# riffusion/riffusion-hobby

Measured on NVIDIA H100. Metric: clips/sec, higher is better.
Workload: dtype f16

## Files before the change

riffusion-hobby_b200/csrc/rf_attn.cu:

```cuda
#include <cuda.h>
#include <cuda_fp16.h>
#include <cuda_runtime.h>

#include <string>

#include "rf_common.h"
#include "rf_tc.cuh"

namespace {

constexpr int TQ = 128;
constexpr int TK = 64;
constexpr int ATTN_THREADS = 256 + 32;

struct AttnParams {
    int Nq, Nk, d, heads;
    int n_tiles;
    float c;
    __half* out;
    long out_pitch;
    int causal;
};

__device__ __forceinline__ uint32_t pack_half2(float a, float b) {
    const __half2 h = __floats2half2_rn(a, b);
    return *reinterpret_cast<const uint32_t*>(&h);
}
__device__ __forceinline__ float ex2(float a) {
    float r;
    asm("ex2.approx.ftz.f32 %0, %1;" : "=f"(r) : "f"(a));
    return r;
}

template <int DPAD, int NV, int NS>
__global__ void __launch_bounds__(ATTN_THREADS, 1)
k_flash_attn(const __grid_constant__ CUtensorMap mapQ, const __grid_constant__ CUtensorMap mapK,
             const __grid_constant__ CUtensorMap mapVt, const AttnParams p) {
    extern __shared__ __align__(1024) uint8_t smem[];
    rf_pdl_trigger();
    constexpr int NSLAB = DPAD / 64;
    constexpr int Q_BYTES = NSLAB * TQ * 128;
    constexpr int K_BYTES = NSLAB * TK * 128;
    constexpr int V_BYTES = ((NV * 128 + 1023) / 1024) * 1024;
    uint8_t* sQ = smem;
    uint8_t* sK = sQ + Q_BYTES;
    uint8_t* sV = sK + NS * K_BYTES;
    uint64_t* bars = reinterpret_cast<uint64_t*>(sV + NS * V_BYTES);
    uint64_t* q_full = bars;
    uint64_t* kv_full = bars + 1;
    uint64_t* kv_empty = kv_full + NS;

    const int warp = threadIdx.x >> 5, lane = threadIdx.x & 31;
    const int q_blk = blockIdx.x, head = blockIdx.y, b = blockIdx.z;
    const int T = p.n_tiles;

    if (threadIdx.x == 0) {
        tc::mbar_init(q_full, 1);
        for (int i = 0; i < NS; ++i) {
            tc::mbar_init(&kv_full[i], 1);
            tc::mbar_init(&kv_empty[i], 256);
        }
        tc::fence_barrier_init();
    }
    __syncthreads();
    rf_pdl_wait();

    if (warp == 8) {
        if (lane != 0) return;
        tc::mbar_expect_tx(q_full, Q_BYTES);
#pragma unroll
        for (int s = 0; s < NSLAB; ++s) tc::tma_load_4d(&mapQ, q_full, sQ + s * TQ * 128, s * 64, q_blk * TQ, head, b);
        for (int j = 0; j < T; ++j) {
            const int st = j % NS;
            tc::mbar_wait(&kv_empty[st], ((j / NS) & 1) ^ 1);
            tc::mbar_expect_tx(&kv_full[st], K_BYTES + NV * 128);
#pragma unroll
            for (int s = 0; s < NSLAB; ++s)
                tc::tma_load_4d(&mapK, &kv_full[st], sK + st * K_BYTES + s * TK * 128, s * 64, j * TK, head, b);
            tc::tma_load_4d(&mapVt, &kv_full[st], sV + st * V_BYTES, j * TK, 0, head, b);
        }
        return;
    }

    const int wg = warp >> 2;
    const int frag_row = wg * 64 + (warp & 3) * 16 + (lane >> 2), frag_col = 2 * (lane & 3);
    const int q0 = q_blk * TQ + frag_row, q1 = q0 + 8;
    const float c = p.c;
    float o[NV / 2];
#pragma unroll
    for (int i = 0; i < NV / 2; ++i) o[i] = 0.f;
    float m0 = -INFINITY, m1 = -INFINITY, l0 = 0.f, l1 = 0.f;
    const uint32_t q_base = tc::smem_u32(sQ) + wg * (64 * 128);
    tc::mbar_wait(q_full, 0);
    for (int j = 0; j < T; ++j) {
        const int st = j % NS;
        tc::mbar_wait(&kv_full[st], (j / NS) & 1);
        float s[TK / 2];
        const uint32_t k_base = tc::smem_u32(sK + st * K_BYTES);
        tc::wgmma_fence();
#pragma unroll
        for (int kk = 0; kk < DPAD / 16; ++kk) {
            const int sl = kk >> 2, k = kk & 3;
            tc::wgmma_ss<TK>(s, tc::make_desc_sw128(q_base + sl * TQ * 128 + k * 32),
                             tc::make_desc_sw128(k_base + sl * TK * 128 + k * 32), kk > 0 ? 1u : 0u);
        }
        tc::wgmma_commit();
        tc::wgmma_wait<0>();
        tc::reg_fence<TK / 2>(s);
        const int kmax0 = p.causal ? min(p.Nk, q0 + 1) : p.Nk, kmax1 = p.causal ? min(p.Nk, q1 + 1) : p.Nk;
        float mt0 = -INFINITY, mt1 = -INFINITY;
#pragma unroll
        for (int i = 0; i < TK / 8; ++i) {
#pragma unroll
            for (int e = 0; e < 2; ++e) {
                const int key = j * TK + 8 * i + frag_col + e;
                if (key >= kmax0) s[4 * i + e] = -INFINITY;
                if (key >= kmax1) s[4 * i + 2 + e] = -INFINITY;
                mt0 = fmaxf(mt0, s[4 * i + e]);
                mt1 = fmaxf(mt1, s[4 * i + 2 + e]);
            }
        }
        mt0 = fmaxf(mt0, __shfl_xor_sync(0xffffffffu, mt0, 1));
        mt0 = fmaxf(mt0, __shfl_xor_sync(0xffffffffu, mt0, 2));
        mt1 = fmaxf(mt1, __shfl_xor_sync(0xffffffffu, mt1, 1));
        mt1 = fmaxf(mt1, __shfl_xor_sync(0xffffffffu, mt1, 2));
        const float mn0 = fmaxf(m0, mt0), mn1 = fmaxf(m1, mt1);
        const float r0 = mn0 == -INFINITY ? 0.f : mn0, r1 = mn1 == -INFINITY ? 0.f : mn1;
        const float f0 = ex2((m0 - r0) * c), f1 = ex2((m1 - r1) * c);
        m0 = mn0;
        m1 = mn1;
        l0 *= f0;
        l1 *= f1;
#pragma unroll
        for (int i = 0; i < NV / 8; ++i) {
            o[4 * i] *= f0;
            o[4 * i + 1] *= f0;
            o[4 * i + 2] *= f1;
            o[4 * i + 3] *= f1;
        }
        const float mc0 = r0 * c, mc1 = r1 * c;
        uint32_t pa[TK / 4];
#pragma unroll
        for (int i = 0; i < TK / 8; ++i) {
            const uint32_t h0 = pack_half2(ex2(fmaf(s[4 * i], c, -mc0)), ex2(fmaf(s[4 * i + 1], c, -mc0)));
            const uint32_t h1 = pack_half2(ex2(fmaf(s[4 * i + 2], c, -mc1)), ex2(fmaf(s[4 * i + 3], c, -mc1)));
            const float2 g0 = __half22float2(*reinterpret_cast<const __half2*>(&h0));
            const float2 g1 = __half22float2(*reinterpret_cast<const __half2*>(&h1));
            l0 += g0.x + g0.y;
            l1 += g1.x + g1.y;
            pa[2 * i] = h0;
            pa[2 * i + 1] = h1;
        }
        const uint32_t v_base = tc::smem_u32(sV + st * V_BYTES);
        tc::wgmma_fence();
#pragma unroll
        for (int kk = 0; kk < TK / 16; ++kk)
            tc::wgmma_rs<NV>(o, pa + 4 * kk, tc::make_desc_sw128(v_base + kk * 32), 1u);
        tc::wgmma_commit();
        tc::wgmma_wait<0>();
        tc::reg_fence<NV / 2>(o);
        tc::mbar_arrive(&kv_empty[st]);
    }
    l0 += __shfl_xor_sync(0xffffffffu, l0, 1);
    l0 += __shfl_xor_sync(0xffffffffu, l0, 2);
    l1 += __shfl_xor_sync(0xffffffffu, l1, 1);
    l1 += __shfl_xor_sync(0xffffffffu, l1, 2);
    const float inv0 = 1.f / l0, inv1 = 1.f / l1;
    __half* dst0 = p.out + (static_cast<long>(b) * p.Nq + q0) * p.out_pitch + head * p.d;
    __half* dst1 = dst0 + 8 * p.out_pitch;
#pragma unroll
    for (int i = 0; i < NV / 8; ++i) {
        const int col = 8 * i + frag_col;
        if (col < p.d) {
            if (q0 < p.Nq) *reinterpret_cast<uint32_t*>(dst0 + col) = pack_half2(o[4 * i] * inv0, o[4 * i + 1] * inv0);
            if (q1 < p.Nq) *reinterpret_cast<uint32_t*>(dst1 + col) = pack_half2(o[4 * i + 2] * inv1, o[4 * i + 3] * inv1);
        }
    }
}

template <int DPAD, int NV, int NS>
int launch_attn(const CUtensorMap& mq, const CUtensorMap& mk, const CUtensorMap& mv, const AttnParams& p, dim3 grid,
                cudaStream_t st) {
    constexpr int NSLAB = DPAD / 64;
    constexpr int V_BYTES = ((NV * 128 + 1023) / 1024) * 1024;
    constexpr size_t smem = static_cast<size_t>(NSLAB) * TQ * 128 + static_cast<size_t>(NS) * (NSLAB * TK * 128 + V_BYTES) +
                            256 + 1024;
    static_assert(smem <= 232448, "shared memory budget (227 KB per block)");
    static rf_dev_once once;
    const cudaError_t aerr = rf_set_smem_once(once, k_flash_attn<DPAD, NV, NS>, int(smem));
    if (aerr != cudaSuccess) return rf_fail(RF_ERR_CUDA, std::string("cudaFuncSetAttribute(k_flash_attn): ") + cudaGetErrorString(aerr));
    RF_LAUNCH_PDL("k_flash_attn", (k_flash_attn<DPAD, NV, NS>), grid, dim3(ATTN_THREADS), smem, st,
                  grid.x * grid.y * grid.z <= 600u, mq, mk, mv, p);
    return RF_OK;
}

}

extern "C" int rf_attention_masked_f16(const void* q, const void* k, const void* vt, void* out, int B, int heads, int Nq,
                                       int Nk, int d, int vt_pitch, float scale, int causal, void* stream) {
    if (causal && (Nk > 128 || d > 112))
        return rf_fail(RF_ERR_UNSUPPORTED, "rf_attention_masked_f16: the causal mask is implemented for Nk <= 128, d <= 112 "
                                           "(the 77-token text encoder)");
    if (!q || !k || !vt || !out || B <= 0 || heads <= 0 || Nq <= 0 || Nk <= 0 || d <= 0 || (d % 8) || vt_pitch < Nk ||
        (vt_pitch % 8))
        return rf_fail(RF_ERR_INVALID, "rf_attention_masked_f16: bad argument");
    if (d > 192) return rf_fail(RF_ERR_UNSUPPORTED, "rf_attention_masked_f16: head dim > 192 (use the GEMM + softmax path)");
    const long C = static_cast<long>(heads) * d;
    const int es[4] = {1, 1, 1, 1};
    CUtensorMap mq, mk, mv;
    {
        const long dims[4] = {d, Nq, heads, B};
        const long str[4] = {1, C, d, static_cast<long>(Nq) * C};
        const int box[4] = {64, TQ, 1, 1};
        int rc = rf_tma_map_f16(&mq, q, dims, str, box, es);
        if (rc) return rc;
    }
    {
        const long dims[4] = {d, Nk, heads, B};
        const long str[4] = {1, C, d, static_cast<long>(Nk) * C};
        const int box[4] = {64, TK, 1, 1};
        int rc = rf_tma_map_f16(&mk, k, dims, str, box, es);
        if (rc) return rc;
    }
    const int NV = d <= 48 ? 48 : d <= 64 ? 64 : d <= 80 ? 80 : d <= 96 ? 96 : d <= 112 ? 112 : d <= 128 ? 128 : d <= 160 ? 160 : 192;
    {
        const long dims[4] = {Nk, d, heads, B};
        const long str[4] = {1, vt_pitch, static_cast<long>(d) * vt_pitch, C * vt_pitch};
        const int box[4] = {TK, NV, 1, 1};
        int rc = rf_tma_map_f16(&mv, vt, dims, str, box, es);
        if (rc) return rc;
    }
    AttnParams p;
    p.Nq = Nq; p.Nk = Nk; p.d = d; p.heads = heads;
    p.n_tiles = (Nk + TK - 1) / TK;
    p.c = scale * 1.4426950408889634f;
    p.out = static_cast<__half*>(out);
    p.out_pitch = C;
    p.causal = causal ? 1 : 0;
    dim3 grid((Nq + TQ - 1) / TQ, heads, B);
    cudaStream_t st = static_cast<cudaStream_t>(stream);
    if (d <= 48) return launch_attn<64, 48, 4>(mq, mk, mv, p, grid, st);
    if (d <= 64) return launch_attn<64, 64, 4>(mq, mk, mv, p, grid, st);
    if (d <= 80) return launch_attn<128, 80, 3>(mq, mk, mv, p, grid, st);
    if (d <= 96) return launch_attn<128, 96, 3>(mq, mk, mv, p, grid, st);
    if (d <= 112) return launch_attn<128, 112, 3>(mq, mk, mv, p, grid, st);
    if (d <= 128) return launch_attn<128, 128, 3>(mq, mk, mv, p, grid, st);
    if (d <= 160) return launch_attn<192, 160, 2>(mq, mk, mv, p, grid, st);
    return launch_attn<192, 192, 2>(mq, mk, mv, p, grid, st);
}
```

Measured before the change: 3.839.

## Parameterize flash attention by warpgroup count and skip padded head-dim work

The kernel is templated on head-dim max and the number of consumer warpgroups. Small head dims (<=64) now use 4 warpgroups and a 256-row Q tile, which halves K/V reloads per query. The QK^T k-loop now runs only up to the real head dim instead of the padded slab width, and masking runs only for causal or ragged tail tiles. The empty barrier now counts per-warp arrivals rather than per-thread ones. In exchange there are more registers and threads per block for small d, and fewer blocks in the grid.

```diff
diff --git a/riffusion-hobby_b200/csrc/rf_attn.cu b/riffusion-hobby_b200/csrc/rf_attn.cu
--- a/riffusion-hobby_b200/csrc/rf_attn.cu
+++ b/riffusion-hobby_b200/csrc/rf_attn.cu
@@ -9,9 +9,7 @@
 
 namespace {
 
-constexpr int TQ = 128;
 constexpr int TK = 64;
-constexpr int ATTN_THREADS = 256 + 32;
 
 struct AttnParams {
     int Nq, Nk, d, heads;
@@ -32,16 +30,30 @@
     return r;
 }
 
-template <int DPAD, int NV, int NS>
-__global__ void __launch_bounds__(ATTN_THREADS, 1)
+template <int DMAX, int NWG, int NS>
+struct AttnCfg {
+    static constexpr int TQ = 64 * NWG;
+    static constexpr int THREADS = 128 * NWG + 32;
+    static constexpr int NSLAB = (DMAX + 63) / 64;
+    static constexpr int KS = (DMAX + 15) / 16;
+    static constexpr int NV = (DMAX + 15) / 16 * 16;
+    static constexpr int Q_BYTES = NSLAB * TQ * 128;
+    static constexpr int K_BYTES = NSLAB * TK * 128;
+    static constexpr int V_BYTES = (NV * 128 + 1023) / 1024 * 1024;
+    static constexpr size_t SMEM = static_cast<size_t>(Q_BYTES) + static_cast<size_t>(NS) * (K_BYTES + V_BYTES) + 256 + 1024;
+    static_assert(SMEM <= 232448, "shared memory budget (227 KB per block)");
+    static_assert(TQ <= 256 && NV <= 256, "TMA box and wgmma N are at most 256");
+};
+
+template <int DMAX, int NWG, int NS>
+__global__ void __launch_bounds__(AttnCfg<DMAX, NWG, NS>::THREADS, 1)
 k_flash_attn(const __grid_constant__ CUtensorMap mapQ, const __grid_constant__ CUtensorMap mapK,
              const __grid_constant__ CUtensorMap mapVt, const AttnParams p) {
+    using Cfg = AttnCfg<DMAX, NWG, NS>;
+    constexpr int TQ = Cfg::TQ, NSLAB = Cfg::NSLAB, KS = Cfg::KS, NV = Cfg::NV;
+    constexpr int Q_BYTES = Cfg::Q_BYTES, K_BYTES = Cfg::K_BYTES, V_BYTES = Cfg::V_BYTES;
     extern __shared__ __align__(1024) uint8_t smem[];
     rf_pdl_trigger();
-    constexpr int NSLAB = DPAD / 64;
-    constexpr int Q_BYTES = NSLAB * TQ * 128;
-    constexpr int K_BYTES = NSLAB * TK * 128;
-    constexpr int V_BYTES = ((NV * 128 + 1023) / 1024) * 1024;
     uint8_t* sQ = smem;
     uint8_t* sK = sQ + Q_BYTES;
     uint8_t* sV = sK + NS * K_BYTES;
@@ -52,20 +64,20 @@
 
     const int warp = threadIdx.x >> 5, lane = threadIdx.x & 31;
     const int q_blk = blockIdx.x, head = blockIdx.y, b = blockIdx.z;
-    const int T = p.n_tiles;
+    const int T = p.n_tiles, d = p.d;
 
     if (threadIdx.x == 0) {
         tc::mbar_init(q_full, 1);
         for (int i = 0; i < NS; ++i) {
             tc::mbar_init(&kv_full[i], 1);
-            tc::mbar_init(&kv_empty[i], 256);
+            tc::mbar_init(&kv_empty[i], 4 * NWG);
         }
         tc::fence_barrier_init();
     }
     __syncthreads();
     rf_pdl_wait();
 
-    if (warp == 8) {
+    if (warp == 4 * NWG) {
         if (lane != 0) return;
         tc::mbar_expect_tx(q_full, Q_BYTES);
 #pragma unroll
@@ -99,7 +111,7 @@
         const uint32_t k_base = tc::smem_u32(sK + st * K_BYTES);
         tc::wgmma_fence();
 #pragma unroll
-        for (int kk = 0; kk < DPAD / 16; ++kk) {
+        for (int kk = 0; kk < KS; ++kk) {
             const int sl = kk >> 2, k = kk & 3;
             tc::wgmma_ss<TK>(s, tc::make_desc_sw128(q_base + sl * TQ * 128 + k * 32),
                              tc::make_desc_sw128(k_base + sl * TK * 128 + k * 32), kk > 0 ? 1u : 0u);
@@ -107,15 +119,23 @@
         tc::wgmma_commit();
         tc::wgmma_wait<0>();
         tc::reg_fence<TK / 2>(s);
-        const int kmax0 = p.causal ? min(p.Nk, q0 + 1) : p.Nk, kmax1 = p.causal ? min(p.Nk, q1 + 1) : p.Nk;
+        if (p.causal || (j + 1) * TK > p.Nk) {
+            const int kmax0 = p.causal ? min(p.Nk, q0 + 1) : p.Nk, kmax1 = p.causal ? min(p.Nk, q1 + 1) : p.Nk;
+#pragma unroll
+            for (int i = 0; i < TK / 8; ++i) {
+#pragma unroll
+                for (int e = 0; e < 2; ++e) {
+                    const int key = j * TK + 8 * i + frag_col + e;
+                    if (key >= kmax0) s[4 * i + e] = -INFINITY;
+                    if (key >= kmax1) s[4 * i + 2 + e] = -INFINITY;
+                }
+            }
+        }
         float mt0 = -INFINITY, mt1 = -INFINITY;
 #pragma unroll
         for (int i = 0; i < TK / 8; ++i) {
 #pragma unroll
             for (int e = 0; e < 2; ++e) {
-                const int key = j * TK + 8 * i + frag_col + e;
-                if (key >= kmax0) s[4 * i + e] = -INFINITY;
-                if (key >= kmax1) s[4 * i + 2 + e] = -INFINITY;
                 mt0 = fmaxf(mt0, s[4 * i + e]);
                 mt1 = fmaxf(mt1, s[4 * i + 2 + e]);
             }
@@ -159,37 +179,57 @@
         tc::wgmma_commit();
         tc::wgmma_wait<0>();
         tc::reg_fence<NV / 2>(o);
-        tc::mbar_arrive(&kv_empty[st]);
+        if (lane == 0) tc::mbar_arrive(&kv_empty[st]);
     }
     l0 += __shfl_xor_sync(0xffffffffu, l0, 1);
     l0 += __shfl_xor_sync(0xffffffffu, l0, 2);
     l1 += __shfl_xor_sync(0xffffffffu, l1, 1);
     l1 += __shfl_xor_sync(0xffffffffu, l1, 2);
     const float inv0 = 1.f / l0, inv1 = 1.f / l1;
-    __half* dst0 = p.out + (static_cast<long>(b) * p.Nq + q0) * p.out_pitch + head * p.d;
+    __half* dst0 = p.out + (static_cast<long>(b) * p.Nq + q0) * p.out_pitch + head * d;
     __half* dst1 = dst0 + 8 * p.out_pitch;
 #pragma unroll
     for (int i = 0; i < NV / 8; ++i) {
         const int col = 8 * i + frag_col;
-        if (col < p.d) {
+        if (col < d) {
             if (q0 < p.Nq) *reinterpret_cast<uint32_t*>(dst0 + col) = pack_half2(o[4 * i] * inv0, o[4 * i + 1] * inv0);
             if (q1 < p.Nq) *reinterpret_cast<uint32_t*>(dst1 + col) = pack_half2(o[4 * i + 2] * inv1, o[4 * i + 3] * inv1);
         }
     }
 }
 
-template <int DPAD, int NV, int NS>
-int launch_attn(const CUtensorMap& mq, const CUtensorMap& mk, const CUtensorMap& mv, const AttnParams& p, dim3 grid,
-                cudaStream_t st) {
-    constexpr int NSLAB = DPAD / 64;
-    constexpr int V_BYTES = ((NV * 128 + 1023) / 1024) * 1024;
-    constexpr size_t smem = static_cast<size_t>(NSLAB) * TQ * 128 + static_cast<size_t>(NS) * (NSLAB * TK * 128 + V_BYTES) +
-                            256 + 1024;
-    static_assert(smem <= 232448, "shared memory budget (227 KB per block)");
+template <int DMAX, int NWG, int NS>
+int launch_attn(const void* q, const void* k, const void* vt, int B, int vt_pitch, const AttnParams& p, cudaStream_t st) {
+    using Cfg = AttnCfg<DMAX, NWG, NS>;
+    const long C = static_cast<long>(p.heads) * p.d;
+    const int es[4] = {1, 1, 1, 1};
+    CUtensorMap mq, mk, mv;
+    {
+        const long dims[4] = {p.d, p.Nq, p.heads, B};
+        const long str[4] = {1, C, p.d, static_cast<long>(p.Nq) * C};
+        const int box[4] = {64, Cfg::TQ, 1, 1};
+        int rc = rf_tma_map_f16(&mq, q, dims, str, box, es);
+        if (rc) return rc;
+    }
+    {
+        const long dims[4] = {p.d, p.Nk, p.heads, B};
+        const long str[4] = {1, C, p.d, static_cast<long>(p.Nk) * C};
+        const int box[4] = {64, TK, 1, 1};
+        int rc = rf_tma_map_f16(&mk, k, dims, str, box, es);
+        if (rc) return rc;
+    }
+    {
+        const long dims[4] = {p.Nk, p.d, p.heads, B};
+        const long str[4] = {1, vt_pitch, static_cast<long>(p.d) * vt_pitch, C * vt_pitch};
+        const int box[4] = {TK, Cfg::NV, 1, 1};
+        int rc = rf_tma_map_f16(&mv, vt, dims, str, box, es);
+        if (rc) return rc;
+    }
+    const dim3 grid((p.Nq + Cfg::TQ - 1) / Cfg::TQ, p.heads, B);
     static rf_dev_once once;
-    const cudaError_t aerr = rf_set_smem_once(once, k_flash_attn<DPAD, NV, NS>, int(smem));
+    const cudaError_t aerr = rf_set_smem_once(once, k_flash_attn<DMAX, NWG, NS>, int(Cfg::SMEM));
     if (aerr != cudaSuccess) return rf_fail(RF_ERR_CUDA, std::string("cudaFuncSetAttribute(k_flash_attn): ") + cudaGetErrorString(aerr));
-    RF_LAUNCH_PDL("k_flash_attn", (k_flash_attn<DPAD, NV, NS>), grid, dim3(ATTN_THREADS), smem, st,
+    RF_LAUNCH_PDL("k_flash_attn", (k_flash_attn<DMAX, NWG, NS>), grid, dim3(Cfg::THREADS), Cfg::SMEM, st,
                   grid.x * grid.y * grid.z <= 600u, mq, mk, mv, p);
     return RF_OK;
 }
@@ -205,46 +245,20 @@
         (vt_pitch % 8))
         return rf_fail(RF_ERR_INVALID, "rf_attention_masked_f16: bad argument");
     if (d > 192) return rf_fail(RF_ERR_UNSUPPORTED, "rf_attention_masked_f16: head dim > 192 (use the GEMM + softmax path)");
-    const long C = static_cast<long>(heads) * d;
-    const int es[4] = {1, 1, 1, 1};
-    CUtensorMap mq, mk, mv;
-    {
-        const long dims[4] = {d, Nq, heads, B};
-        const long str[4] = {1, C, d, static_cast<long>(Nq) * C};
-        const int box[4] = {64, TQ, 1, 1};
-        int rc = rf_tma_map_f16(&mq, q, dims, str, box, es);
-        if (rc) return rc;
-    }
-    {
-        const long dims[4] = {d, Nk, heads, B};
-        const long str[4] = {1, C, d, static_cast<long>(Nk) * C};
-        const int box[4] = {64, TK, 1, 1};
-        int rc = rf_tma_map_f16(&mk, k, dims, str, box, es);
-        if (rc) return rc;
-    }
-    const int NV = d <= 48 ? 48 : d <= 64 ? 64 : d <= 80 ? 80 : d <= 96 ? 96 : d <= 112 ? 112 : d <= 128 ? 128 : d <= 160 ? 160 : 192;
-    {
-        const long dims[4] = {Nk, d, heads, B};
-        const long str[4] = {1, vt_pitch, static_cast<long>(d) * vt_pitch, C * vt_pitch};
-        const int box[4] = {TK, NV, 1, 1};
-        int rc = rf_tma_map_f16(&mv, vt, dims, str, box, es);
-        if (rc) return rc;
-    }
     AttnParams p;
     p.Nq = Nq; p.Nk = Nk; p.d = d; p.heads = heads;
     p.n_tiles = (Nk + TK - 1) / TK;
     p.c = scale * 1.4426950408889634f;
     p.out = static_cast<__half*>(out);
-    p.out_pitch = C;
+    p.out_pitch = static_cast<long>(heads) * d;
     p.causal = causal ? 1 : 0;
-    dim3 grid((Nq + TQ - 1) / TQ, heads, B);
     cudaStream_t st = static_cast<cudaStream_t>(stream);
-    if (d <= 48) return launch_attn<64, 48, 4>(mq, mk, mv, p, grid, st);
-    if (d <= 64) return launch_attn<64, 64, 4>(mq, mk, mv, p, grid, st);
-    if (d <= 80) return launch_attn<128, 80, 3>(mq, mk, mv, p, grid, st);
-    if (d <= 96) return launch_attn<128, 96, 3>(mq, mk, mv, p, grid, st);
-    if (d <= 112) return launch_attn<128, 112, 3>(mq, mk, mv, p, grid, st);
-    if (d <= 128) return launch_attn<128, 128, 3>(mq, mk, mv, p, grid, st);
-    if (d <= 160) return launch_attn<192, 160, 2>(mq, mk, mv, p, grid, st);
-    return launch_attn<192, 192, 2>(mq, mk, mv, p, grid, st);
-}
+    if (d <= 48) return launch_attn<48, 4, 4>(q, k, vt, B, vt_pitch, p, st);
+    if (d <= 64) return launch_attn<64, 4, 4>(q, k, vt, B, vt_pitch, p, st);
+    if (d <= 80) return launch_attn<80, 2, 3>(q, k, vt, B, vt_pitch, p, st);
+    if (d <= 96) return launch_attn<96, 2, 3>(q, k, vt, B, vt_pitch, p, st);
+    if (d <= 112) return launch_attn<112, 2, 3>(q, k, vt, B, vt_pitch, p, st);
+    if (d <= 128) return launch_attn<128, 2, 3>(q, k, vt, B, vt_pitch, p, st);
+    if (d <= 160) return launch_attn<160, 2, 2>(q, k, vt, B, vt_pitch, p, st);
+    return launch_attn<192, 2, 2>(q, k, vt, B, vt_pitch, p, st);
+}
```

Measured after the change: 3.943, median of 6. 2.7% higher.
